# nilsbore/gp_compressor

Hardware: AMD Instinct MI355X
Metric: patches/sec (compress+predict) (higher is better)
Workload: dtype f64; 1 GPU; C2 room scan: 8192 patches x 256 pts per GPU, RBF + Gaussian noise, dense Cholesky fit + predictive mean on the 20x20 grid (m=400); patches_per_gpu=8192, points_per_patch=256, grid_points=400, parallelism=1 GPU, kernel=dense_mfma_w1

## Files before the change

### gp_compressor_amd/csrc/dense_mfma_w1.hip

```cpp
#include <cstdio>
#include <cstdlib>
#include <type_traits>

#include "gpc_device.h"
#include "gpc_internal.h"
#include "mfma_tile.h"

#define W1_NPAD_MAX 512
#define W1_C 4
#define W1_NDT 10
#define W1_NT_OF(npad) ((npad) / 16)
#define W1_TRI_OF(npad) (W1_NT_OF(npad) * (W1_NT_OF(npad) + 1) / 2)
#define W1_TILE(i, j) (((size_t)(i) * (size_t)((i) + 1) / 2 + (size_t)(j)) * MF_IMG)


struct W1Params {
    DenseArgs a;
    double c_exp;
    double pivot_tol;
    double cs, noise_u, sfp, a_out;
    double* ws;
    double* linvt;
    int export_factor;
    unsigned long long* stamps;
};
#define W1_NPH 12
#ifdef W1_STAMPS
#define W1_STAMP(ph)                                                                                                 \
    do {                                                                                                             \
        __builtin_amdgcn_sched_barrier(0);                                                                           \
        const unsigned long long t_now_ = __builtin_amdgcn_s_memtime();                                              \
        st_acc_[ph] += t_now_ - t_prev_;                                                                             \
        t_prev_ = t_now_;                                                                                            \
        __builtin_amdgcn_sched_barrier(0);                                                                           \
    } while (0)
#else
#define W1_STAMP(ph) do { } while (0)
#endif

#define W1_LDS_SYNC()                                                                                                \
    do {                                                                                                             \
        __builtin_amdgcn_fence(__ATOMIC_SEQ_CST, "wavefront");                                                       \
        __builtin_amdgcn_wave_barrier();                                                                             \
    } while (0)

template <int A, int B, typename F>
__device__ static __forceinline__ void w1_static_for(F&& f)
{
    if constexpr (A < B) {
        f(std::integral_constant<int, A>{});
        w1_static_for<A + 1, B>(f);
    }
}
__host__ __device__ constexpr int w1_stream_col(int q)
{
    int kk = 0;
    while ((kk + 1) * (kk + 2) / 2 <= q) ++kk;
    return kk;
}
#define W1_BW 20

__device__ static __forceinline__ d4 w1_mfma4_neg(d4 a, d4 b, d4 acc)
{
#pragma unroll
    for (int s = 0; s < 4; ++s) acc = __builtin_amdgcn_mfma_f64_16x16x4f64(a[s], b[s], acc, 0, 0, 1);
    return acc;
}
__device__ static __forceinline__ d4 w1_trsm(d4 lv, d4 src)
{
    const d4 z4 = d4{0.0, 0.0, 0.0, 0.0};
    d4 D = __builtin_amdgcn_mfma_f64_16x16x4f64(lv[0], src[0], z4, 0, 0, 0);
    D = __builtin_amdgcn_mfma_f64_16x16x4f64(lv[1], src[1], D, 0, 0, 0);
    D = __builtin_amdgcn_mfma_f64_16x16x4f64(lv[2], src[2], D, 0, 0, 0);
    return __builtin_amdgcn_mfma_f64_16x16x4f64(lv[3], src[3], D, 0, 0, 0);
}

template <int MODE, int CNT, bool DIAG>
__device__ static __forceinline__ void w1_gram_row(d4 (&v)[W1_C], const double* px0, const double* px1, const double* T, double sf, bool scale_sf,
                                                   double cexp, double noise, bool dbl, int n, int r, int c0, int lr, int lg)
{
    const int pi = MF_TS * r + lr;
    const double xi0 = px0[pi], xi1 = px1[pi];
#pragma unroll
    for (int t = 0; t < CNT; ++t) {
#pragma unroll
        for (int q = 0; q < 4; ++q) {
            const int pj = MF_TS * (c0 + t) + lg + 4 * q;
            const double d0 = xi0 - px0[pj], d1 = xi1 - px1[pj];
            const double sq = __builtin_fma(d0, d0, d1 * d1);
            v[t][q] = MODE == 0 ? gpc_exp_neg(cexp * sq, T) : gpc_expm_poly<MODE == 1 ? 7 : 5>(sq);
        }
    }
    if (scale_sf) {
#pragma unroll
        for (int t = 0; t < CNT; ++t)
#pragma unroll
            for (int q = 0; q < 4; ++q) v[t][q] *= sf;
    }
    if constexpr (DIAG) {
#pragma unroll
        for (int q = 0; q < 4; ++q) {
            double d = v[CNT - 1][q] + noise;
            if (dbl) d += noise;
            v[CNT - 1][q] = (lr == lg + 4 * q) ? d : v[CNT - 1][q];
        }
    }
    if (MF_TS * (r + 1) > n || MF_TS * (c0 + CNT) > n) {
#pragma unroll
        for (int t = 0; t < CNT; ++t) {
#pragma unroll
            for (int q = 0; q < 4; ++q) {
                const int pj = MF_TS * (c0 + t) + lg + 4 * q;
                if (pi >= n || pj >= n) v[t][q] = (pi == pj) ? 1.0 : 0.0;
            }
        }
    }
}

template <int W1_NPAD>
__global__ __launch_bounds__(64, 2) void dense_w1_kernel(W1Params g)
{
    constexpr int W1_NT = W1_NT_OF(W1_NPAD), W1_TRI = W1_TRI_OF(W1_NPAD);
    __shared__ __attribute__((aligned(16))) double T[GPC_EXP_TABLE_SIZE];
    __shared__ __attribute__((aligned(16))) double px0[W1_NPAD], px1[W1_NPAD], zv[W1_NPAD];
    __shared__ __attribute__((aligned(16))) double rsbuf[32], wsc[32];
    __shared__ __attribute__((aligned(16))) double LinvC[W1_C * MF_IMG];

    const DenseArgs& A = g.a;
    int lane = threadIdx.x;
    int lr = lane & 15, lg = lane >> 4;
#define W1_FRESH_LANE()                                                                                              \
    do {                                                                                                             \
        lane = mf_opaque(lane);                                                                                      \
        lr = lane & 15;                                                                                              \
        lg = lane >> 4;                                                                                              \
    } while (0)
    const int m = A.m;
    const double sf = A.prm.sigmaf_sq, cexp = g.c_exp;
    const bool dbl = A.prm.ref_double_noise != 0;
    const int patch = blockIdx.x;
    double* Lt = g.ws + (size_t)patch * W1_TRI * MF_IMG;
    double* LinvTg = g.linvt + (size_t)patch * W1_NT * MF_IMG;

    gpc_exp_table_init(T);
    {
        const int o = __builtin_amdgcn_readfirstlane(A.off[patch]);
        const int n = __builtin_amdgcn_readfirstlane(A.off[patch + 1]) - o;
        double* fs = A.f_star + (size_t)patch * m;
        __syncthreads();
        if (n <= 0 || n > W1_NPAD) {
            for (int p = lane; p < m; p += 64) fs[p] = (n == 0) ? 0.0 : __builtin_nan("");
            if (lane == 0 && A.status) A.status[patch] = (n == 0) ? GPC_STATUS_OK : GPC_STATUS_NAN;
            return;
        }
        const int nt = __builtin_amdgcn_readfirstlane((n + MF_TS - 1) / MF_TS);
#ifdef W1_STAMPS
        unsigned long long st_acc_[W1_NPH] = {};
        unsigned long long t_prev_ = __builtin_amdgcn_s_memtime();
#endif

        const double xo0 = A.x0[o], xo1 = A.x1[o];
        double qr0[W1_NPAD / 64], qr1[W1_NPAD / 64];
        double mn0 = xo0, mx0 = xo0, mn1 = xo1, mx1 = xo1;
#pragma unroll
        for (int u = 0; u < W1_NPAD / 64; ++u) {
            const int i = lane + 64 * u;
            const bool live = i < n;
            qr0[u] = live ? A.x0[o + i] : xo0;
            qr1[u] = live ? A.x1[o + i] : xo1;
            mn0 = __builtin_fmin(mn0, qr0[u]); mx0 = __builtin_fmax(mx0, qr0[u]);
            mn1 = __builtin_fmin(mn1, qr1[u]); mx1 = __builtin_fmax(mx1, qr1[u]);
            zv[i] = live ? A.y[o + i] : 0.0;
        }
#pragma unroll
        for (int o_ = 32; o_ > 0; o_ >>= 1) {
            mn0 = __builtin_fmin(mn0, __shfl_xor(mn0, o_, 64)); mx0 = __builtin_fmax(mx0, __shfl_xor(mx0, o_, 64));
            mn1 = __builtin_fmin(mn1, __shfl_xor(mn1, o_, 64)); mx1 = __builtin_fmax(mx1, __shfl_xor(mx1, o_, 64));
        }
        int mode_g, mode_p;
        {
            const bool nan_box = !((mx0 - mn0) + (mx1 - mn1) < __builtin_inf());
            const double rx = mx0 - mn0, ry = mx1 - mn1;
            const double tg = nan_box ? __builtin_inf() : -cexp * __builtin_fma(rx, rx, ry * ry);
            const double hb = 0.5 * A.grid_res;
            const double bx = hb + __builtin_fmax(__builtin_fabs(mn0), __builtin_fabs(mx0));
            const double by = hb + __builtin_fmax(__builtin_fabs(mn1), __builtin_fabs(mx1));
            const double bq = __builtin_fmax(bx, by);
            const double tp = nan_box ? __builtin_inf() : -cexp * (bq * bq);
            mode_g = __builtin_amdgcn_readfirstlane(tg <= GPC_EXP_TINY_MAX ? 2 : tg <= GPC_EXP_SMALL_MAX ? 1 : 0);
            mode_p = __builtin_amdgcn_readfirstlane(tp <= GPC_EXP_TINY_MAX ? 2 : tp <= GPC_EXP_SMALL_MAX ? 1 : 0);
            if (mode_g == 0) mode_p = 0;
        }
        const bool scaled = mode_g > 0;
        {
            const double cs = scaled ? g.cs : 1.0;
            const double co0 = scaled ? xo0 : 0.0, co1 = scaled ? xo1 : 0.0;
#pragma unroll
            for (int u = 0; u < W1_NPAD / 64; ++u) {
                const int i = lane + 64 * u;
                const bool live = i < n;
                px0[i] = live ? cs * (qr0[u] - co0) : 0.0;
                px1[i] = live ? cs * (qr1[u] - co1) : 0.0;
            }
        }
        const bool scale_sf = g.export_factor != 0;
        const double noise_u = g.noise_u, ptol = g.pivot_tol;
        W1_LDS_SYNC();
#define W1_GRAM_ROW(v, CNT, DIAG, r, c0)                                                                              \
    do {                                                                                                             \
        if (mode_g == 2) w1_gram_row<2, CNT, DIAG>(v, px0, px1, T, sf, scale_sf, cexp, noise_u, dbl, n, r, c0, lr, lg);   \
        else if (mode_g == 1) w1_gram_row<1, CNT, DIAG>(v, px0, px1, T, sf, scale_sf, cexp, noise_u, dbl, n, r, c0, lr, lg); \
        else w1_gram_row<0, CNT, DIAG>(v, px0, px1, T, sf, scale_sf, cexp, noise_u, dbl, n, r, c0, lr, lg);            \
    } while (0)

        auto bw_step = [&](auto P, const d4 img, d4& pa) __attribute__((always_inline)) {
            constexpr int q = decltype(P)::value;
            constexpr int kk = w1_stream_col(q), t = q - kk * (kk + 1) / 2;
            if (kk < nt) {
                const int k = nt - 1 - kk;
                if constexpr (t < kk) {
                    const double a_ = zv[MF_TS * (k + 1 + t) + lr];
                    pa += img * a_;
                } else {
                    d4 ub = d4{0.0, 0.0, 0.0, 0.0};
                    if constexpr (kk > 0) {
                        const double tot = mf_row_reduce4(pa, lr);
                        if ((lr & 3) == 0) wsc[lg + 4 * (lr >> 2)] = tot;
                        W1_LDS_SYNC();
                        if (lr == 0) {
#pragma unroll
                            for (int q4 = 0; q4 < 4; ++q4) ub[q4] = zv[MF_TS * k + lg + 4 * q4] - wsc[lg + 4 * q4];
                        }
                    } else {
                        if (lr == 0) {
#pragma unroll
                            for (int q4 = 0; q4 < 4; ++q4) ub[q4] = zv[MF_TS * k + lg + 4 * q4];
                        }
                    }
                    const d4 al = w1_trsm(img, ub);
                    W1_LDS_SYNC();
                    if (lr == 0) {
#pragma unroll
                        for (int r = 0; r < 4; ++r) zv[MF_TS * k + lg + 4 * r] = al[r];
                    }
                    W1_LDS_SYNC();
                    pa = d4{0.0, 0.0, 0.0, 0.0};
                }
            }
        };
        bool bad = false;
        W1_STAMP(0);
#define W1_BLOCK_ROW(bi, kb, nb)                                                                                     \
    do {                                                                                                             \
        if ((bi) < (nb)) {                                                                                           \
            d4 gv[W1_C];                                                                                             \
            W1_GRAM_ROW(gv, (bi) + 1, true, (kb) + (bi), (kb));                                                      \
            _Pragma("unroll") for (int bc = 0; bc <= (bi); ++bc) tacc[(bi) * ((bi) + 1) / 2 + bc] = gv[bc];           \
        } else {                                                                                                     \
            _Pragma("unroll") for (int bc = 0; bc <= (bi); ++bc) tacc[(bi) * ((bi) + 1) / 2 + bc] = d4{0.0, 0.0, 0.0, 0.0}; \
        }                                                                                                            \
    } while (0)
#define W1_BLOCK_INIT(kb, nb)                                                                                        \
    do {                                                                                                             \
        _Pragma("unroll") for (int i = 0; i < W1_C; ++i) part[i] = 0.0;                                              \
                                             \
        __builtin_amdgcn_sched_barrier(0);                                                                           \
        W1_BLOCK_ROW(3, kb, nb);                                                                                     \
        __builtin_amdgcn_sched_barrier(0);                                                                           \
        W1_BLOCK_ROW(2, kb, nb);                                                                                     \
        __builtin_amdgcn_sched_barrier(0);                                                                           \
        W1_BLOCK_ROW(1, kb, nb);                                                                                     \
        __builtin_amdgcn_sched_barrier(0);                                                                           \
        W1_BLOCK_ROW(0, kb, nb);                                                                                     \
        __builtin_amdgcn_sched_barrier(0);                                                                           \
    } while (0)
        W1_STAMP(1);
        for (int k = 0;; k += W1_C) {
            const int nc = min(W1_C, nt - k);
            const int kl = k - 1;
            const bool last_step = k + W1_C >= nt;
            (void)last_step;
            W1_FRESH_LANE();
            const double* rrow[W1_C];
#pragma unroll
            for (int i = 0; i < W1_C; ++i) rrow[i] = Lt + W1_TILE(k + min(i, nc - 1), 0);
            d4 tacc[W1_NDT];
            double part[W1_C];
            d4 op[2][W1_C];
#pragma unroll
            for (int i = 0; i < W1_C; ++i) op[0][i] = op[1][i] = d4{0.0, 0.0, 0.0, 0.0};
            if (k > 0) {
#pragma unroll
                for (int i = 0; i < W1_C; ++i) op[0][i] = mf_img_load(rrow[i], lane);
            }
            W1_BLOCK_INIT(k, nc);
            for (int j = 0; j < k; j += 2) {
#pragma unroll
                for (int h = 0; h < 2; ++h) {
                    const int jn = min(j + h + 1, kl);
#pragma unroll
                    for (int i = 0; i < W1_C; ++i) op[h ^ 1][i] = mf_img_load(rrow[i] + (size_t)jn * MF_IMG, lane);
#pragma unroll
                    for (int d = 0; d < W1_NDT; ++d) {
                        const int bi = d >= 6 ? 3 : d >= 3 ? 2 : d >= 1 ? 1 : 0, bc = d - bi * (bi + 1) / 2;
                        if (bi < nc) tacc[d] = w1_mfma4_neg(op[h][bc], op[h][bi], tacc[d]);
                    }
                    const double* zq = zv + MF_TS * (j + h) + lg;
                    const double z0 = zq[0], z1 = zq[4], z2 = zq[8], z3 = zq[12];
#pragma unroll
                    for (int c = 0; c < W1_C; ++c) part[c] += (op[h][c][0] * z0 + op[h][c][1] * z1) + (op[h][c][2] * z2 + op[h][c][3] * z3);
                }
            }
            W1_STAMP(2);
            W1_FRESH_LANE();
            d4 Lb[W1_C * (W1_C - 1) / 2];
#pragma unroll
            for (int q = 0; q < W1_C * (W1_C - 1) / 2; ++q) Lb[q] = d4{0.0, 0.0, 0.0, 0.0};
            bool ok = mf_diag_factor_c(tacc[0], rsbuf, LinvC, LinvTg + (size_t)k * MF_IMG, ptol, lane);
            W1_LDS_SYNC();
            if (g.export_factor) mf_img_store(Lt + W1_TILE(k, k), lane, mf_img_load(LinvC, lane));
#pragma unroll
            for (int i = 1; i < W1_C; ++i) {
                if (ok && i < nc) {
#pragma unroll
                    for (int c = 0; c < i; ++c) {
                        d4 Tt = tacc[i * (i + 1) / 2 + c];
#pragma unroll
                        for (int c2 = 0; c2 < c; ++c2) Tt = w1_mfma4_neg(Lb[c * (c - 1) / 2 + c2], Lb[i * (i - 1) / 2 + c2], Tt);
                        const d4 lvc = mf_img_load(LinvC + c * MF_IMG, mf_opaque(lane));
                        const d4 L = w1_trsm(lvc, Tt);
                        Lb[i * (i - 1) / 2 + c] = L;
                        mf_img_store(Lt + W1_TILE(k + i, k + c), lane, L);
                    }
                    d4 Dii = tacc[i * (i + 1) / 2 + i];
#pragma unroll
                    for (int c = 0; c < i; ++c) Dii = w1_mfma4_neg(Lb[i * (i - 1) / 2 + c], Lb[i * (i - 1) / 2 + c], Dii);
                    ok = mf_diag_factor_c(Dii, rsbuf, LinvC + i * MF_IMG, LinvTg + (size_t)(k + i) * MF_IMG, ptol, lane);
                    W1_LDS_SYNC();
                    if (g.export_factor) mf_img_store(Lt + W1_TILE(k + i, k + i), lane, mf_img_load(LinvC + i * MF_IMG, mf_opaque(lane)));
                }
            }
            if (!ok) { bad = true; break; }
            W1_STAMP(3);
            W1_FRESH_LANE();
#pragma unroll
            for (int c = 0; c < W1_C; ++c) {
                if (c < nc) {
                    const int pj = MF_TS * (k + c) + lr;
                    double pp = part[c];
#pragma unroll
                    for (int c2 = 0; c2 < c; ++c2) {
                        const d4 lb = Lb[c * (c - 1) / 2 + c2];
                        const double* zq = zv + MF_TS * (k + c2) + lg;
                        pp += (lb[0] * zq[0] + lb[1] * zq[4]) + (lb[2] * zq[8] + lb[3] * zq[12]);
                    }
                    pp += __shfl_xor(pp, 16, 64);
                    pp += __shfl_xor(pp, 32, 64);
                    const double yv = zv[pj];
                    W1_LDS_SYNC();
                    if (lg == 0) zv[pj] = yv - pp;
                    W1_LDS_SYNC();
                    const d4 lv = mf_img_load(LinvC + c * MF_IMG, mf_opaque(lane));
                    const double* tq = zv + MF_TS * (k + c) + lg;
                    double zz = (lv[0] * tq[0] + lv[1] * tq[4]) + (lv[2] * tq[8] + lv[3] * tq[12]);
                    zz += __shfl_xor(zz, 16, 64);
                    zz += __shfl_xor(zz, 32, 64);
                    W1_LDS_SYNC();
                    if (lg == 0) zv[pj] = zz;
                    W1_LDS_SYNC();
                }
            }
            W1_STAMP(4);
            const int rows_tot = nt - (k + nc);
            if (rows_tot == 0) {
                __syncthreads();
                break;
            }
            if (k > 0) __syncthreads();
            const int npass = (rows_tot + 3) / 4;
            const int klp = k - 1;
            if (k == 0) {
                for (int pi_ = 0; pi_ < npass; ++pi_) {
                    const int first_row0 = (pi_ + 1 < npass) ? 4 * (pi_ + 1) : 0;
                    const int np4 = min(4, rows_tot - first_row0);
                    W1_FRESH_LANE();
                    d4 cy[W1_C][4];
#pragma unroll
                    for (int t = 0; t < 4; ++t) {
                        const int r_ = W1_C + first_row0 + min(t, np4 - 1);
                        d4 gv[W1_C];
                        W1_GRAM_ROW(gv, 2, false, r_, 0);
                        cy[0][t] = gv[0]; cy[1][t] = gv[1];
                        __builtin_amdgcn_sched_barrier(0);
                        W1_GRAM_ROW(gv, 2, false, r_, 2);
                        cy[2][t] = gv[0]; cy[3][t] = gv[1];
                        __builtin_amdgcn_sched_barrier(0);
                    }
                    W1_STAMP(5);
#pragma unroll
                    for (int c = 0; c < W1_C; ++c) {
                        const d4 lv = mf_img_load(LinvC + c * MF_IMG, mf_opaque(lane));
#pragma unroll
                        for (int t = 0; t < 4; ++t) {
#pragma unroll
                            for (int c2 = 0; c2 < c; ++c2) cy[c][t] = w1_mfma4_neg(Lb[c * (c - 1) / 2 + c2], cy[c2][t], cy[c][t]);
                            cy[c][t] = w1_trsm(lv, cy[c][t]);
                            if (t < np4) mf_img_store(Lt + W1_TILE(W1_C + first_row0 + t, c), lane, cy[c][t]);
                        }
                    }
                    W1_STAMP(7);
                }
            }
            if (k > 0) {
                for (int pi_ = 0; pi_ < npass; ++pi_) {
                    const int first_row = (pi_ + 1 < npass) ? 4 * (pi_ + 1) : 0;
                    const int np4 = min(4, rows_tot - first_row);
                    W1_FRESH_LANE();
                    d4 cy[W1_C][4];
                    int rr[4];
                    const double* rw_[4];
#pragma unroll
                    for (int t = 0; t < 4; ++t) {
                        rr[t] = k + W1_C + first_row + min(t, np4 - 1);
                        rw_[t] = Lt + W1_TILE(rr[t], 0);
                    }
                    d4 A2[2][W1_C], B[4];
#pragma unroll
                    for (int c = 0; c < W1_C; ++c) A2[0][c] = mf_img_load(rrow[c], lane);
#pragma unroll
                    for (int t = 0; t < 4; ++t) B[t] = mf_img_load(rw_[t], lane);
#pragma unroll
                    for (int t = 0; t < 4; ++t) {
                        d4 gv[W1_C];
                        W1_GRAM_ROW(gv, 2, false, rr[t], k);
                        cy[0][t] = gv[0]; cy[1][t] = gv[1];
                        __builtin_amdgcn_sched_barrier(0);
                        W1_GRAM_ROW(gv, 2, false, rr[t], k + 2);
                        cy[2][t] = gv[0]; cy[3][t] = gv[1];
                        __builtin_amdgcn_sched_barrier(0);
                    }
                    W1_STAMP(5);
                    d4 Lq[W1_C * (W1_C - 1) / 2];
#define W1_PASS_J(st, jn, PREFETCH)                                                                                  \
    do {                                                                                                             \
                                      \
        if (PREFETCH) {                                                                                              \
            _Pragma("unroll") for (int c = 0; c < W1_C; ++c) A2[(st) ^ 1][c] = mf_img_load(rrow[c] + (size_t)(jn) * MF_IMG, lane); \
        }                                                                                                            \
        __builtin_amdgcn_sched_barrier(0);                                                                           \
        _Pragma("unroll") for (int t = 0; t < 4; ++t) {                                                              \
            _Pragma("unroll") for (int c = 0; c < W1_C; ++c) cy[c][t] = w1_mfma4_neg(A2[st][c], B[t], cy[c][t]);      \
            __builtin_amdgcn_sched_barrier(0);                                                                       \
            if (PREFETCH) B[t] = mf_img_load(rw_[t] + (size_t)(jn) * MF_IMG, lane);                                    \
            else {      \
                if (t < 3) Lq[t] = mf_img_load(Lt + W1_TILE(k + (t == 0 ? 1 : 2), k + (t == 2 ? 1 : 0)), lane);      \
                else {                                                                                               \
                    _Pragma("unroll") for (int c2 = 0; c2 < 3; ++c2) Lq[3 + c2] = mf_img_load(Lt + W1_TILE(k + 3, k + c2), lane); \
                }                                                                                                    \
            }                                                                                                        \
            __builtin_amdgcn_sched_barrier(0);                                                                       \
        }                                                                                                            \
    } while (0)
                    for (int j = 0; j + 2 < k; j += 2) {
                        W1_PASS_J(0, j + 1, true);
                        W1_PASS_J(1, j + 2, true);
                    }
                    W1_PASS_J(0, klp, true);
                    W1_PASS_J(1, klp, false);
#undef W1_PASS_J
                    W1_STAMP(6);
                    W1_FRESH_LANE();
#pragma unroll
                    for (int c = 0; c < W1_C; ++c) {
                        const d4 lv = mf_img_load(LinvC + c * MF_IMG, mf_opaque(lane));
#pragma unroll
                        for (int t = 0; t < 4; ++t) {
#pragma unroll
                            for (int c2 = 0; c2 < c; ++c2) cy[c][t] = w1_mfma4_neg(Lq[c * (c - 1) / 2 + c2], cy[c2][t], cy[c][t]);
                            cy[c][t] = w1_trsm(lv, cy[c][t]);
                            if (t < np4) mf_img_store(Lt + W1_TILE(rr[t], k + c), lane, cy[c][t]);
                        }
                    }
                    W1_STAMP(7);
                }
            }
            __syncthreads();
            W1_STAMP(8);
        }
#undef W1_BLOCK_INIT
#undef W1_BLOCK_ROW

        if (bad) {
            for (int p = lane; p < m; p += 64) fs[p] = __builtin_nan("");
            if (A.alpha_out)
                for (int i = lane; i < n; i += 64) A.alpha_out[o + i] = __builtin_nan("");
            if (lane == 0 && A.status) A.status[patch] = GPC_STATUS_NOT_SPD;
            return;
        }

        {
            W1_FRESH_LANE();
            constexpr int NP = W1_NPAD / MF_TS;
            constexpr int SLEN = NP * (NP + 1) / 2;
            d4 win[W1_BW];
            auto stream_addr = [&](auto P) __attribute__((always_inline)) -> const double* {
                constexpr int q = decltype(P)::value;
                constexpr int kk = w1_stream_col(q), t = q - kk * (kk + 1) / 2;
                const int kq = max(nt - 1 - kk, 0);
                const double* ad = (t < kk) ? Lt + W1_TILE(kq + 1 + t, kq) : LinvTg + (size_t)kq * MF_IMG;
                return kk < nt ? ad : Lt;
            };
            w1_static_for<0, W1_BW>([&](auto P) __attribute__((always_inline)) {
                constexpr int q = decltype(P)::value;
                win[q] = mf_img_load_nt(stream_addr(P), lane);
            });
            d4 pa = d4{0.0, 0.0, 0.0, 0.0};
            w1_static_for<0, SLEN>([&](auto P) __attribute__((always_inline)) {
                constexpr int q = decltype(P)::value;
                bw_step(P, win[q % W1_BW], pa);
                if constexpr (q + W1_BW < SLEN) {
                    win[q % W1_BW] = mf_img_load_nt(stream_addr(std::integral_constant<int, q + W1_BW>{}), lane);
                }
            });
        }
        W1_STAMP(9);
        double* av = zv;
        if (A.alpha_out)
            for (int i = lane; i < n; i += 64) A.alpha_out[o + i] = av[i] * g.a_out;

        W1_FRESH_LANE();
        if (m <= 0) {
        } else if (A.xs0 == nullptr && A.grid_sz <= 32) {
            const int sz = A.grid_sz;
            const double res = A.grid_res;
            d4 P[2][2];
#pragma unroll
            for (int mt = 0; mt < 2; ++mt)
#pragma unroll
                for (int nl = 0; nl < 2; ++nl) P[mt][nl] = d4{0.0, 0.0, 0.0, 0.0};
            double gqx[2], gqy[2];
            const double cs = scaled ? g.cs : 1.0, co0 = scaled ? A.x0[o] : 0.0, co1 = scaled ? A.x1[o] : 0.0;
            const double argc = scaled ? -1.0 : cexp, sfp = g.sfp;
#pragma unroll
            for (int h = 0; h < 2; ++h) {
                const double gq = res * (((double)(16 * h + lr) + 0.5) / (double)sz - 0.5);
                gqx[h] = cs * (gq - co0);
                gqy[h] = cs * (gq - co1);
            }
            auto predict_loop = [&](auto mode_tag) __attribute__((always_inline)) {
                constexpr int MP = decltype(mode_tag)::value;
                for (int ibase = 0; ibase < n; ibase += 32) {
#pragma unroll
                    for (int s = 0; s < 8; ++s) {
                        const int i = ibase + 4 * s + lg;
                        const int ic = min(i, W1_NPAD - 1);
                        const double al = (i < n) ? sfp * av[ic] : 0.0;
                        const double xi0 = px0[ic], xi1 = px1[ic];
                        double ea[2], eb[2];
#pragma unroll
                        for (int h = 0; h < 2; ++h) {
                            const double dy = gqy[h] - xi1, dx = gqx[h] - xi0;
                            if constexpr (MP == 0) {
                                ea[h] = gpc_exp_neg(argc * (dy * dy), T);
                                eb[h] = gpc_exp_neg(argc * (dx * dx), T) * al;
                            } else {
                                ea[h] = gpc_expm_poly<MP == 1 ? 7 : 5>(dy * dy);
                                eb[h] = gpc_expm_poly<MP == 1 ? 7 : 5>(dx * dx) * al;
                            }
                        }
#pragma unroll
                        for (int nl = 0; nl < 2; ++nl)
#pragma unroll
                            for (int mt = 0; mt < 2; ++mt)
                                P[mt][nl] = __builtin_amdgcn_mfma_f64_16x16x4f64(ea[mt], eb[nl], P[mt][nl], 0, 0, 0);
                    }
                }
            };
            if (mode_p == 2) predict_loop(std::integral_constant<int, 2>{});
            else if (mode_p == 1) predict_loop(std::integral_constant<int, 1>{});
            else predict_loop(std::integral_constant<int, 0>{});
#pragma unroll
            for (int mt = 0; mt < 2; ++mt)
#pragma unroll
                for (int nl = 0; nl < 2; ++nl)
#pragma unroll
                    for (int r = 0; r < 4; ++r) {
                        const int py = 16 * mt + lg + 4 * r, pxx = 16 * nl + lr;
                        if (py < sz && pxx < sz) fs[py * sz + pxx] = P[mt][nl][r];
                    }
        } else {
            const double cs = scaled ? g.cs : 1.0, co0 = scaled ? A.x0[o] : 0.0, co1 = scaled ? A.x1[o] : 0.0;
            const double argc = scaled ? -1.0 : cexp, sfp = g.sfp;
            for (int p = lane; p < m; p += 64) {
                double q0, q1;
                if (A.xs0) {
                    q0 = A.xs0[p];
                    q1 = A.xs1[p];
                } else {
                    const int gx = p % A.grid_sz, gy = p / A.grid_sz;
                    q0 = A.grid_res * (((double)gx + 0.5) / (double)A.grid_sz - 0.5);
                    q1 = A.grid_res * (((double)gy + 0.5) / (double)A.grid_sz - 0.5);
                }
                q0 = cs * (q0 - co0);
                q1 = cs * (q1 - co1);
                double s_ = 0.0;
                for (int i = 0; i < n; ++i) {
                    const double d0 = px0[i] - q0, d1 = px1[i] - q1;
                    s_ += gpc_exp_neg(argc * __builtin_fma(d0, d0, d1 * d1), T) * av[i];
                }
                fs[p] = sfp * s_;
            }
        }
        if (lane == 0 && A.status) A.status[patch] = GPC_STATUS_OK;
#ifdef W1_STAMPS
        W1_STAMP(10);
        if (g.stamps && lane == 0)
            for (int q_ = 0; q_ < W1_NPH; ++q_) atomicAdd(g.stamps + q_, st_acc_[q_]);
#endif
    }
}

static int w1_npad(const DenseArgs& a) { return a.n_max <= 256 ? 256 : W1_NPAD_MAX; }

bool dense_w1_supported(const DenseArgs& a)
{
    if (a.v_star) return a.n_max <= 256 && a.ny == 1 && !a.sel && a.xs0 != nullptr;
    return a.n_max <= W1_NPAD_MAX && a.ny == 1 && !a.sel;
}

#define W1_MAX_SLOTS 8192
static int w1_chunk(const DenseArgs& a, int cap_in)
{
    const char* e = getenv("GPC_W1_SLOTS");
    int cap = e && atoi(e) > 0 ? atoi(e) : W1_MAX_SLOTS;
    if (cap_in > 0 && cap_in < cap) cap = cap_in;
    return a.P < cap ? a.P : cap;
}

size_t dense_w1_ws_bytes(const gpc_ctx* ctx, const DenseArgs& a, int* grid_out, int cap)
{
    (void)ctx;
    const int grid = w1_chunk(a, cap);
    if (grid_out) *grid_out = grid;
    const int npad = w1_npad(a);
    return sizeof(double) * ((size_t)(W1_TRI_OF(npad) + W1_NT_OF(npad)) * MF_IMG * (size_t)grid + (a.v_star ? (size_t)a.n_total : 0));
}

int dense_w1_launch(gpc_ctx* ctx, const DenseArgs& a_in, int grid)
{
    DenseArgs a = a_in;
    double* v_star = a.v_star;
    a.v_star = nullptr;
    W1Params g;
    g.c_exp = (double)(-0.5f) / a.prm.l_sq;
    g.ws = reinterpret_cast<double*>(static_cast<char*>(ctx->ws) + ctx->ws_off);
    const int npad = w1_npad(a);
    g.linvt = g.ws + (size_t)W1_TRI_OF(npad) * MF_IMG * (size_t)grid;
    g.export_factor = v_star ? 1 : 0;
    const double sf = a.prm.sigmaf_sq;
    const bool unit = !v_star;
    g.cs = sqrt(-g.c_exp);
    g.noise_u = unit ? a.prm.noise / sf : a.prm.noise;
    g.pivot_tol = GPC_PIVOT_RTOL * (unit ? 1.0 + a.prm.noise / sf : sf + a.prm.noise);
    g.sfp = unit ? 1.0 : sf;
    g.a_out = unit ? 1.0 / sf : 1.0;
    g.stamps = nullptr;
    if (v_star) {
        a.m = 0;
        if (!a.alpha_out) a.alpha_out = g.linvt + (size_t)W1_NT_OF(npad) * MF_IMG * (size_t)grid;
    }
    ctx->last_dense_kernel = v_star ? "dense_mfma_w1 + dense_variance" : npad == 256 ? "dense_mfma_w1" : "dense_mfma_w1_512";
#ifdef W1_STAMPS
    if (getenv("GPC_W1_STAMPS")) {
        GPC_HIP(ctx, hipMalloc(&g.stamps, sizeof(unsigned long long) * W1_NPH));
        GPC_HIP(ctx, hipMemsetAsync(g.stamps, 0, sizeof(unsigned long long) * W1_NPH, ctx->stream));
    }
#endif
    for (int base = 0; base < a.P; base += grid) {
        const int cnt = a.P - base < grid ? a.P - base : grid;
        g.a = a;
        g.a.P = cnt;
        g.a.off = a.off + base;
        g.a.f_star = a.f_star ? a.f_star + (size_t)base * a.ny * a_in.m : nullptr;
        g.a.status = a.status ? a.status + base : nullptr;
        if (npad == 256) hipLaunchKernelGGL((dense_w1_kernel<256>), dim3(cnt), dim3(64), 0, ctx->stream, g);
        else hipLaunchKernelGGL((dense_w1_kernel<W1_NPAD_MAX>), dim3(cnt), dim3(64), 0, ctx->stream, g);
        GPC_HIP(ctx, hipGetLastError());
        if (v_star) {
            DenseArgs av = g.a;
            av.m = a_in.m;
            const int rc = dense_variance_launch(ctx, av, W1_NT_OF(256), g.ws, a.alpha_out, v_star + (size_t)base * a_in.m);
            if (rc != GPC_OK) return rc;
        }
    }
#ifdef W1_STAMPS
    if (g.stamps) {
        unsigned long long h[W1_NPH];
        GPC_HIP(ctx, hipStreamSynchronize(ctx->stream));
        GPC_HIP(ctx, hipMemcpy(h, g.stamps, sizeof(h), hipMemcpyDeviceToHost));
        (void)hipFree(g.stamps);
        static const char* names[W1_NPH] = {"load", "sweep gram", "sweep loop", "chain", "forward", "pass gram", "pass loop", "pass trsm",
                                            "step fence", "backward", "predict", ""};
        unsigned long long tot = 0;
        for (int q = 0; q < W1_NPH; ++q) tot += h[q];
        fprintf(stderr, "[GPC_W1_STAMPS] mean s_memtime ticks per patch (total %.0f)\n", (double)tot / a.P);
        for (int q = 0; q < 11; ++q) fprintf(stderr, "  %-12s %9.0f  %5.1f %%\n", names[q], (double)h[q] / a.P, 100.0 * h[q] / tot);
    }
#endif
    return GPC_OK;
}
```

Measured before the change: 5.550 million patches/s.

## Carry next block's first row pass in registers into the diagonal update

The blocked right-looking Cholesky is restructured. Each step's first panel row pass, covering the rows of the next diagonal block, is now deferred and run at the start of the next iteration. Its results stay in registers (cy) and seed the diagonal syrk accumulation and the z dot products directly, instead of being stored and reloaded from global memory. The row pass becomes a shared lambda, and lane id is recomputed through mbcnt inline asm to control register pressure and rematerialisation. This adds control-flow complexity and register pressure, and changes the pass ordering and which rows the update loops cover.

After: 5.372 million patches/s. -3.2%, worse.

```diff
diff --git a/gp_compressor_amd/csrc/dense_mfma_w1.hip b/gp_compressor_amd/csrc/dense_mfma_w1.hip
--- a/gp_compressor_amd/csrc/dense_mfma_w1.hip
+++ b/gp_compressor_amd/csrc/dense_mfma_w1.hip
@@ -60,6 +60,18 @@
 }
 #define W1_BW 20
 
+__device__ static __forceinline__ int w1_lane_id()
+{
+    int l;
+    asm volatile("v_mbcnt_lo_u32_b32 %0, -1, 0\n\tv_mbcnt_hi_u32_b32 %0, -1, %0" : "=v"(l));
+    return l & 63;
+}
+__device__ static __forceinline__ d4 w1_zero4()
+{
+    double z = 0.0;
+    asm volatile("" : "+v"(z));
+    return d4{z, z, z, z};
+}
 __device__ static __forceinline__ d4 w1_mfma4_neg(d4 a, d4 b, d4 acc)
 {
 #pragma unroll
@@ -127,11 +139,11 @@
     __shared__ __attribute__((aligned(16))) double LinvC[W1_C * MF_IMG];
 
     const DenseArgs& A = g.a;
-    int lane = threadIdx.x;
+    int lane = w1_lane_id();
     int lr = lane & 15, lg = lane >> 4;
 #define W1_FRESH_LANE()                                                                                              \
     do {                                                                                                             \
-        lane = mf_opaque(lane);                                                                                      \
+        lane = w1_lane_id();                                                                                         \
         lr = lane & 15;                                                                                              \
         lg = lane >> 4;                                                                                              \
     } while (0)
@@ -148,7 +160,9 @@
         const int n = __builtin_amdgcn_readfirstlane(A.off[patch + 1]) - o;
         double* fs = A.f_star + (size_t)patch * m;
         __syncthreads();
+        W1_FRESH_LANE();
         if (n <= 0 || n > W1_NPAD) {
+            W1_FRESH_LANE();
             for (int p = lane; p < m; p += 64) fs[p] = (n == 0) ? 0.0 : __builtin_nan("");
             if (lane == 0 && A.status) A.status[patch] = (n == 0) ? GPC_STATUS_OK : GPC_STATUS_NAN;
             return;
@@ -255,14 +269,11 @@
         if ((bi) < (nb)) {                                                                                           \
             d4 gv[W1_C];                                                                                             \
             W1_GRAM_ROW(gv, (bi) + 1, true, (kb) + (bi), (kb));                                                      \
-            _Pragma("unroll") for (int bc = 0; bc <= (bi); ++bc) tacc[(bi) * ((bi) + 1) / 2 + bc] = gv[bc];           \
-        } else {                                                                                                     \
-            _Pragma("unroll") for (int bc = 0; bc <= (bi); ++bc) tacc[(bi) * ((bi) + 1) / 2 + bc] = d4{0.0, 0.0, 0.0, 0.0}; \
+            _Pragma("unroll") for (int bc = 0; bc <= (bi); ++bc) tacc[(bi) * ((bi) + 1) / 2 + bc] += gv[bc];          \
         }                                                                                                            \
     } while (0)
 #define W1_BLOCK_INIT(kb, nb)                                                                                        \
     do {                                                                                                             \
-        _Pragma("unroll") for (int i = 0; i < W1_C; ++i) part[i] = 0.0;                                              \
                                              \
         __builtin_amdgcn_sched_barrier(0);                                                                           \
         W1_BLOCK_ROW(3, kb, nb);                                                                                     \
@@ -274,48 +285,150 @@
         W1_BLOCK_ROW(0, kb, nb);                                                                                     \
         __builtin_amdgcn_sched_barrier(0);                                                                           \
     } while (0)
+        auto row_pass = [&](auto carried_tag, d4 (&cy)[W1_C][4], const int kb, const int r0, const int np4) __attribute__((always_inline)) {
+            constexpr bool CARRIED = decltype(carried_tag)::value;
+            W1_FRESH_LANE();
+            int rr[4];
+            const double* rw_[4];
+            const double* cw_[W1_C];
+#pragma unroll
+            for (int t = 0; t < 4; ++t) {
+                rr[t] = r0 + min(t, np4 - 1);
+                rw_[t] = Lt + W1_TILE(rr[t], 0);
+            }
+#pragma unroll
+            for (int c = 0; c < W1_C; ++c) cw_[c] = Lt + W1_TILE(kb + c, 0);
+            d4 A2[2][W1_C], B[4];
+#pragma unroll
+            for (int c = 0; c < W1_C; ++c) A2[0][c] = mf_img_load(cw_[c], lane);
+#pragma unroll
+            for (int t = 0; t < 4; ++t) B[t] = mf_img_load(rw_[t], lane);
+#pragma unroll
+            for (int t = 0; t < 4; ++t) {
+                d4 gv[W1_C];
+                W1_GRAM_ROW(gv, 2, false, rr[t], kb);
+                cy[0][t] = gv[0]; cy[1][t] = gv[1];
+                __builtin_amdgcn_sched_barrier(0);
+                W1_GRAM_ROW(gv, 2, false, rr[t], kb + 2);
+                cy[2][t] = gv[0]; cy[3][t] = gv[1];
+                __builtin_amdgcn_sched_barrier(0);
+            }
+            W1_STAMP(5);
+            d4 Lq[W1_C * (W1_C - 1) / 2];
+#define W1_LQ_LOAD(t)                                                                                                \
+    do {                                                                                                             \
+        if ((t) < 3) Lq[t] = mf_img_load(Lt + W1_TILE(kb + ((t) == 0 ? 1 : 2), kb + ((t) == 2 ? 1 : 0)), lane);      \
+        else {                                                                                                       \
+            _Pragma("unroll") for (int c2 = 0; c2 < 3; ++c2) Lq[3 + c2] = mf_img_load(Lt + W1_TILE(kb + 3, kb + c2), lane); \
+        }                                                                                                            \
+    } while (0)
+#define W1_PASS_J(st, jn, PREFETCH)                                                                                  \
+    do {                                                                                                             \
+                                      \
+        if (PREFETCH) {                                                                                              \
+            _Pragma("unroll") for (int c = 0; c < W1_C; ++c) A2[(st) ^ 1][c] = mf_img_load(cw_[c] + (size_t)(jn) * MF_IMG, lane); \
+        }                                                                                                            \
+        __builtin_amdgcn_sched_barrier(0);                                                                           \
+        _Pragma("unroll") for (int t = 0; t < 4; ++t) {                                                              \
+            _Pragma("unroll") for (int c = 0; c < W1_C; ++c) cy[c][t] = w1_mfma4_neg(A2[st][c], B[t], cy[c][t]);      \
+            __builtin_amdgcn_sched_barrier(0);                                                                       \
+            if (PREFETCH) B[t] = mf_img_load(rw_[t] + (size_t)(jn) * MF_IMG, lane);                                    \
+            else if (!CARRIED) W1_LQ_LOAD(t);   \
+            __builtin_amdgcn_sched_barrier(0);                                                                       \
+        }                                                                                                            \
+    } while (0)
+            if (kb > 0) {
+                const int klp = kb - 1;
+                for (int j = 0; j + 2 < kb; j += 2) {
+                    W1_PASS_J(0, j + 1, true);
+                    W1_PASS_J(1, j + 2, true);
+                }
+                W1_PASS_J(0, klp, true);
+                W1_PASS_J(1, klp, false);
+            }
+#undef W1_PASS_J
+            W1_STAMP(6);
+            W1_FRESH_LANE();
+            if constexpr (CARRIED) {
+#pragma unroll
+                for (int t = 0; t < 4; ++t) W1_LQ_LOAD(t);
+            }
+#undef W1_LQ_LOAD
+#pragma unroll
+            for (int c = 0; c < W1_C; ++c) {
+                const d4 lv = mf_img_load(LinvC + c * MF_IMG, mf_opaque(lane));
+#pragma unroll
+                for (int t = 0; t < 4; ++t) {
+#pragma unroll
+                    for (int c2 = 0; c2 < c; ++c2) cy[c][t] = w1_mfma4_neg(Lq[c * (c - 1) / 2 + c2], cy[c2][t], cy[c][t]);
+                    cy[c][t] = w1_trsm(lv, cy[c][t]);
+                    if (t < np4) mf_img_store(Lt + W1_TILE(rr[t], kb + c), lane, cy[c][t]);
+                }
+            }
+            W1_STAMP(7);
+        };
         W1_STAMP(1);
         for (int k = 0;; k += W1_C) {
             const int nc = min(W1_C, nt - k);
-            const int kl = k - 1;
-            const bool last_step = k + W1_C >= nt;
-            (void)last_step;
-            W1_FRESH_LANE();
-            const double* rrow[W1_C];
-#pragma unroll
-            for (int i = 0; i < W1_C; ++i) rrow[i] = Lt + W1_TILE(k + min(i, nc - 1), 0);
             d4 tacc[W1_NDT];
             double part[W1_C];
-            d4 op[2][W1_C];
-#pragma unroll
-            for (int i = 0; i < W1_C; ++i) op[0][i] = op[1][i] = d4{0.0, 0.0, 0.0, 0.0};
+#pragma unroll
+            for (int i = 0; i < W1_C; ++i) part[i] = 0.0;
             if (k > 0) {
-#pragma unroll
-                for (int i = 0; i < W1_C; ++i) op[0][i] = mf_img_load(rrow[i], lane);
-            }
-            W1_BLOCK_INIT(k, nc);
-            for (int j = 0; j < k; j += 2) {
-#pragma unroll
-                for (int h = 0; h < 2; ++h) {
-                    const int jn = min(j + h + 1, kl);
-#pragma unroll
-                    for (int i = 0; i < W1_C; ++i) op[h ^ 1][i] = mf_img_load(rrow[i] + (size_t)jn * MF_IMG, lane);
+                d4 cy[W1_C][4];
+                row_pass(std::true_type{}, cy, k - W1_C, k, nc);
+                const int ks = k - W1_C;
+                const int kl = ks - 1;
+                const double* rrow[W1_C];
+#pragma unroll
+                for (int i = 0; i < W1_C; ++i) rrow[i] = Lt + W1_TILE(k + min(i, nc - 1), 0);
+                d4 op[2][W1_C];
+#pragma unroll
+                for (int c = 0; c < W1_C; ++c) {
 #pragma unroll
                     for (int d = 0; d < W1_NDT; ++d) {
                         const int bi = d >= 6 ? 3 : d >= 3 ? 2 : d >= 1 ? 1 : 0, bc = d - bi * (bi + 1) / 2;
-                        if (bi < nc) tacc[d] = w1_mfma4_neg(op[h][bc], op[h][bi], tacc[d]);
-                    }
-                    const double* zq = zv + MF_TS * (j + h) + lg;
+                        tacc[d] = w1_mfma4_neg(cy[c][bc], cy[c][bi], c == 0 ? d4{0.0, 0.0, 0.0, 0.0} : tacc[d]);
+                    }
+                    const double* zq = zv + MF_TS * (ks + c) + lg;
                     const double z0 = zq[0], z1 = zq[4], z2 = zq[8], z3 = zq[12];
 #pragma unroll
-                    for (int c = 0; c < W1_C; ++c) part[c] += (op[h][c][0] * z0 + op[h][c][1] * z1) + (op[h][c][2] * z2 + op[h][c][3] * z3);
-                }
-            }
+                    for (int t = 0; t < W1_C; ++t) part[t] += (cy[c][t][0] * z0 + cy[c][t][1] * z1) + (cy[c][t][2] * z2 + cy[c][t][3] * z3);
+                    __builtin_amdgcn_sched_barrier(0);
+                    if (c == 1) {
+#pragma unroll
+                        for (int i = 0; i < W1_C; ++i) op[0][i] = op[1][i] = mf_img_load(rrow[i], lane);
+                        __builtin_amdgcn_sched_barrier(0);
+                    }
+                }
+                for (int j = 0; j < ks; j += 2) {
+#pragma unroll
+                    for (int h = 0; h < 2; ++h) {
+                        const int jn = min(j + h + 1, kl);
+#pragma unroll
+                        for (int i = 0; i < W1_C; ++i) op[h ^ 1][i] = mf_img_load(rrow[i] + (size_t)jn * MF_IMG, lane);
+#pragma unroll
+                        for (int d = 0; d < W1_NDT; ++d) {
+                            const int bi = d >= 6 ? 3 : d >= 3 ? 2 : d >= 1 ? 1 : 0, bc = d - bi * (bi + 1) / 2;
+                            if (bi < nc) tacc[d] = w1_mfma4_neg(op[h][bc], op[h][bi], tacc[d]);
+                        }
+                        const double* zq = zv + MF_TS * (j + h) + lg;
+                        const double z0 = zq[0], z1 = zq[4], z2 = zq[8], z3 = zq[12];
+#pragma unroll
+                        for (int c = 0; c < W1_C; ++c) part[c] += (op[h][c][0] * z0 + op[h][c][1] * z1) + (op[h][c][2] * z2 + op[h][c][3] * z3);
+                    }
+                }
+            } else {
+#pragma unroll
+                for (int d = 0; d < W1_NDT; ++d) tacc[d] = w1_zero4();
+            }
+            W1_FRESH_LANE();
+            W1_BLOCK_INIT(k, nc);
             W1_STAMP(2);
             W1_FRESH_LANE();
             d4 Lb[W1_C * (W1_C - 1) / 2];
 #pragma unroll
-            for (int q = 0; q < W1_C * (W1_C - 1) / 2; ++q) Lb[q] = d4{0.0, 0.0, 0.0, 0.0};
+            for (int q = 0; q < W1_C * (W1_C - 1) / 2; ++q) Lb[q] = w1_zero4();
             bool ok = mf_diag_factor_c(tacc[0], rsbuf, LinvC, LinvTg + (size_t)k * MF_IMG, ptol, lane);
             W1_LDS_SYNC();
             if (g.export_factor) mf_img_store(Lt + W1_TILE(k, k), lane, mf_img_load(LinvC, lane));
@@ -377,11 +490,8 @@
                 break;
             }
             if (k > 0) __syncthreads();
-            const int npass = (rows_tot + 3) / 4;
-            const int klp = k - 1;
             if (k == 0) {
-                for (int pi_ = 0; pi_ < npass; ++pi_) {
-                    const int first_row0 = (pi_ + 1 < npass) ? 4 * (pi_ + 1) : 0;
+                for (int first_row0 = 4; first_row0 < rows_tot; first_row0 += 4) {
                     const int np4 = min(4, rows_tot - first_row0);
                     W1_FRESH_LANE();
                     d4 cy[W1_C][4];
@@ -412,76 +522,9 @@
                 }
             }
             if (k > 0) {
-                for (int pi_ = 0; pi_ < npass; ++pi_) {
-                    const int first_row = (pi_ + 1 < npass) ? 4 * (pi_ + 1) : 0;
-                    const int np4 = min(4, rows_tot - first_row);
-                    W1_FRESH_LANE();
+                for (int first_row = 4; first_row < rows_tot; first_row += 4) {
                     d4 cy[W1_C][4];
-                    int rr[4];
-                    const double* rw_[4];
-#pragma unroll
-                    for (int t = 0; t < 4; ++t) {
-                        rr[t] = k + W1_C + first_row + min(t, np4 - 1);
-                        rw_[t] = Lt + W1_TILE(rr[t], 0);
-                    }
-                    d4 A2[2][W1_C], B[4];
-#pragma unroll
-                    for (int c = 0; c < W1_C; ++c) A2[0][c] = mf_img_load(rrow[c], lane);
-#pragma unroll
-                    for (int t = 0; t < 4; ++t) B[t] = mf_img_load(rw_[t], lane);
-#pragma unroll
-                    for (int t = 0; t < 4; ++t) {
-                        d4 gv[W1_C];
-                        W1_GRAM_ROW(gv, 2, false, rr[t], k);
-                        cy[0][t] = gv[0]; cy[1][t] = gv[1];
-                        __builtin_amdgcn_sched_barrier(0);
-                        W1_GRAM_ROW(gv, 2, false, rr[t], k + 2);
-                        cy[2][t] = gv[0]; cy[3][t] = gv[1];
-                        __builtin_amdgcn_sched_barrier(0);
-                    }
-                    W1_STAMP(5);
-                    d4 Lq[W1_C * (W1_C - 1) / 2];
-#define W1_PASS_J(st, jn, PREFETCH)                                                                                  \
-    do {                                                                                                             \
-                                      \
-        if (PREFETCH) {                                                                                              \
-            _Pragma("unroll") for (int c = 0; c < W1_C; ++c) A2[(st) ^ 1][c] = mf_img_load(rrow[c] + (size_t)(jn) * MF_IMG, lane); \
-        }                                                                                                            \
-        __builtin_amdgcn_sched_barrier(0);                                                                           \
-        _Pragma("unroll") for (int t = 0; t < 4; ++t) {                                                              \
-            _Pragma("unroll") for (int c = 0; c < W1_C; ++c) cy[c][t] = w1_mfma4_neg(A2[st][c], B[t], cy[c][t]);      \
-            __builtin_amdgcn_sched_barrier(0);                                                                       \
-            if (PREFETCH) B[t] = mf_img_load(rw_[t] + (size_t)(jn) * MF_IMG, lane);                                    \
-            else {      \
-                if (t < 3) Lq[t] = mf_img_load(Lt + W1_TILE(k + (t == 0 ? 1 : 2), k + (t == 2 ? 1 : 0)), lane);      \
-                else {                                                                                               \
-                    _Pragma("unroll") for (int c2 = 0; c2 < 3; ++c2) Lq[3 + c2] = mf_img_load(Lt + W1_TILE(k + 3, k + c2), lane); \
-                }                                                                                                    \
-            }                                                                                                        \
-            __builtin_amdgcn_sched_barrier(0);                                                                       \
-        }                                                                                                            \
-    } while (0)
-                    for (int j = 0; j + 2 < k; j += 2) {
-                        W1_PASS_J(0, j + 1, true);
-                        W1_PASS_J(1, j + 2, true);
-                    }
-                    W1_PASS_J(0, klp, true);
-                    W1_PASS_J(1, klp, false);
-#undef W1_PASS_J
-                    W1_STAMP(6);
-                    W1_FRESH_LANE();
-#pragma unroll
-                    for (int c = 0; c < W1_C; ++c) {
-                        const d4 lv = mf_img_load(LinvC + c * MF_IMG, mf_opaque(lane));
-#pragma unroll
-                        for (int t = 0; t < 4; ++t) {
-#pragma unroll
-                            for (int c2 = 0; c2 < c; ++c2) cy[c][t] = w1_mfma4_neg(Lq[c * (c - 1) / 2 + c2], cy[c2][t], cy[c][t]);
-                            cy[c][t] = w1_trsm(lv, cy[c][t]);
-                            if (t < np4) mf_img_store(Lt + W1_TILE(rr[t], k + c), lane, cy[c][t]);
-                        }
-                    }
-                    W1_STAMP(7);
+                    row_pass(std::false_type{}, cy, k, k + W1_C + first_row, min(4, rows_tot - first_row));
                 }
             }
             __syncthreads();
@@ -491,6 +534,7 @@
 #undef W1_BLOCK_ROW
 
         if (bad) {
+            W1_FRESH_LANE();
             for (int p = lane; p < m; p += 64) fs[p] = __builtin_nan("");
             if (A.alpha_out)
                 for (int i = lane; i < n; i += 64) A.alpha_out[o + i] = __builtin_nan("");
```
